# yyssys/MH-SpGEMM

Measured on AMD Instinct MI355X. Metric: GFLOPS (2·flop(A,B)/t) for C=A·A on 16matrix.txt; HBM GB/s vs roofline, higher is better.
Workload: dtype f64; 1 GPU; cant.mtx A*A (synthetic:cant-like), device-resident A -> device-resident sorted C; matrix=cant, rows=62451, nnzA=4325625, nnzC=17508231, parallelism=single GPU

## Files before the change

include/mhspgemm.h:

```cpp
#ifndef MHSPGEMM_H
#define MHSPGEMM_H
#include <stddef.h>
#include <stdint.h>

#ifdef __cplusplus
extern "C" {
#endif

#define MHS_ABI_VERSION 10

typedef enum mhs_status {
    MHS_OK = 0,
    MHS_ERR_HIP = 1,
    MHS_ERR_OOM = 2,
    MHS_ERR_INVALID = 3,
    MHS_ERR_OVERFLOW = 4,
    MHS_ERR_IO = 5
} mhs_status;

typedef struct mhs_csr {
    int32_t M, N, nnz;
    int32_t *ptr;
    int32_t *col;
    double *val;
// ... 4 lines not shown
    double Form_mask_matrix_B;
    double symbolic_binning;
    double Calculate_C_nnz;
    double numeric_binning;
    double Malloc_C_col_val;
    double Numeric;
    double total_ref;
    double total_e2e;
    uint64_t flop;
    int64_t nnzC;
    int32_t sym_bins[16];
    int32_t num_bins[16];
} mhs_timing;

typedef struct mhs_ctx mhs_ctx;

int mhs_ctx_create(mhs_ctx **ctx, int device);
void mhs_ctx_destroy(mhs_ctx *ctx);
const char *mhs_last_error(const mhs_ctx *ctx);
int mhs_ctx_set_stream(mhs_ctx *ctx, void *hip_stream);
int mhs_ctx_trim(mhs_ctx *ctx);

typedef enum mhs_option { MHS_OPT_SYNC = 1, MHS_OPT_NUMERIC_EVENTS = 2, MHS_OPT_MEM_BUDGET = 3,
                           MHS_OPT_TINY_FIRST_ROWS = 4, MHS_OPT_SPECULATE = 5 } mhs_option;
int mhs_ctx_set_option(mhs_ctx *ctx, int option, int value);
long long mhs_ctx_chunked_calls(const mhs_ctx *ctx);
typedef enum mhs_stat { MHS_STAT_CHUNKED = 0, MHS_STAT_SPLIT = 1, MHS_STAT_SYM_FORK = 2, MHS_STAT_NFT = 3,
                        MHS_STAT_NEAR = 4, MHS_STAT_MULTI_STREAM = 5, MHS_STAT_SPEC = 6, MHS_STAT_SPEC_MISS = 7,
                        MHS_STAT_SPEC_SKIPPED = 8 } mhs_stat;
long long mhs_ctx_stat(const mhs_ctx *ctx, int which);
int mhs_ctx_numeric_ms(mhs_ctx *ctx, float *out, int n);

int mhs_probe_conflicts(mhs_ctx *ctx, uint64_t *count);

int mhs_spgemm(mhs_ctx *ctx, const mhs_csr *A, const mhs_csr *B, mhs_csr *C, mhs_timing *t);

typedef struct mhs_values_plan mhs_values_plan;

int mhs_values_plan_create(mhs_ctx *ctx, const mhs_csr *A, const mhs_csr *B, const mhs_csr *C,
                           mhs_values_plan **plan);
int mhs_spgemm_values(mhs_ctx *ctx, mhs_values_plan *plan, const double *Aval, const double *Bval,
                      double *Cval, double *ms);
typedef struct mhs_values_info {
    int32_t rows[8];
    int64_t products, nnzC, plan_bytes;
} mhs_values_info;
int mhs_values_plan_info(const mhs_values_plan *plan, mhs_values_info *info);
// ... 35 lines not shown
```

mh-spgemm_amd/csrc/mhs_api.cpp:

```cpp
#include "mhs_internal.hpp"
#include "mhs_owner.hpp"
#include "../../include/mhspgemm.h"

#include <algorithm>
#include <chrono>
#include <cstdio>
#include <cstdlib>
#include <cstring>
#include <string>
#include <unordered_map>
#include <vector>

using namespace mhs;

struct mhs_ctx {
    int device = 0;
    hipStream_t own_stream = nullptr;
    hipStream_t stream = nullptr;
    std::string err;
    char* ws = nullptr;
    size_t ws_bytes = 0;
    char* gscratch = nullptr;
    size_t gscratch_bytes = 0;
    Stats* h_stats = nullptr;
// ... 28 lines not shown
    std::vector<std::pair<void*, size_t>> pool;
    hipEvent_t stream_ev = nullptr;
    static constexpr int NAUX = 7;
    int num_streams = 4;
    hipStream_t aux[NAUX] = {};
    hipEvent_t fork_ev = nullptr, join_ev[NAUX] = {};
    hipEvent_t split_ev = nullptr;
    struct PlanKey {
        const void* p[6];
        long long M, N, MB, nnzA, nnzB, gen;
        int near, nft, mc_list, pad;
        bool operator==(const PlanKey& o) const { return memcmp(this, &o, sizeof *this) == 0; }
    };
    bool spec = true;
    bool plan_valid = false;
    PlanKey plan_key{};
    Stats plan_h{};
    long long gen = 0;
    int* d_go = nullptr;
    bool spec_fork = false;
    bool spec_fork_rare = true;
    bool fork_common_first = true;
    int spec_nss = mhs_ctx::NAUX + 1;
};

struct mhs_values_plan {
    int device = 0;
    ValPattern pat{};
    long long nnzA = 0, nnzB = 0, nnzC = 0, products = 0;
    char* mem = nullptr;
    size_t mem_bytes = 0;
    int* lists = nullptr;
    int list_off[VAL_NCLASS] = {};
    ValCounts counts{};
    ValPlan plan{};
    hipEvent_t ev[2] = {};
};

namespace {
constexpr int VAL_STATUS_INTS = 8;
}

namespace {

int fail(mhs_ctx* ctx, int code, const std::string& what) {
    if (ctx) ctx->err = what;
// ... 270 lines not shown
    if (rc) return rc;
    memcpy(&h, (const void*)&ctx->pub->stats, sizeof(Stats));
    ctx->stats_zero = true;
    ++ctx->front_passes;
    return MHS_OK;
}

constexpr int NUM_GLOBAL_GRID = 128;
#ifndef MHS_MULTI_FLOP_LOG2
#define MHS_MULTI_FLOP_LOG2 22
#endif

#ifndef MHS_SPLIT_FLOP_LOG2
#define MHS_SPLIT_FLOP_LOG2 24
#endif

int numeric_streams(const mhs_ctx* ctx, const Stats& h) {
    const int nl = numeric_launches(h);
    return (nl >= 3 && h.flop >= (1ull << MHS_MULTI_FLOP_LOG2)) ? std::min(ctx->num_streams, nl) : 1;
}

enum NumPhase { NUM_ALL = 0, NUM_SPEC_A = 1, NUM_SPEC_B = 2 };

NumShape num_shape(const Csr& a, const Csr& b, const Work& w, bool split) {
    return NumShape{a.M, a.nnz, b.nnz, w.bx_on, w.sc_col != nullptr, split, NUM_GLOBAL_GRID};
}

int run_numeric(mhs_ctx* ctx, const Csr& a, const Csr& b, const Work& w, const Stats& h, const mhs_csr& out,
                NumPlan& plan, hipEvent_t ev0 = nullptr, hipEvent_t ev1 = nullptr, int phase = NUM_ALL) {
    hipStream_t s = ctx->stream;
    hipStream_t ss[mhs_ctx::NAUX + 1] = {s};
    int nss = numeric_streams(ctx, h);
    if (w.go) nss = std::min(nss, ctx->spec_nss);
    for (int i = 1; i < nss; ++i) ss[i] = ctx->aux[i - 1];
    const bool first = phase != NUM_SPEC_B, last = phase != NUM_SPEC_A;
    if (phase == NUM_SPEC_B && nss == 1) return MHS_OK;
    if (first && nss > 1 && ev0) MHS_HIP(hipEventRecord(ev0, s));
    if (first && nss > 1) MHS_HIP(hipEventRecord(ctx->fork_ev, s));
    if (first) {
        const bool want_split = nss > 1 && ctx->split && h.flop >= (1ull << MHS_SPLIT_FLOP_LOG2);
        const bool split = want_split && launch_split_bins(w, h, a.M, out.ptr, s, ctx->dense_span_max);
        if (split) MHS_HIP(hipEventRecord(ctx->split_ev, s));
        ctx->stat[MHS_STAT_SPLIT] += split;
        ctx->stat[MHS_STAT_MULTI_STREAM] += nss > 1;
        plan = plan_numeric(h, num_shape(a, b, w, split));
    }
    const NumPointers np{a, b, w, out.ptr, out.col, out.val, ctx->dense_span_max};
    hipError_t fe = hipSuccess;
    bool forked = false;
    int used = 0;
    auto fork = [&]() {
        forked = true;
        for (int i = 1; i < nss && fe == hipSuccess; ++i) fe = hipStreamWaitEvent(ss[i], ctx->fork_ev, 0);
    };
    for (int i = 0; i < plan.n; ++i) {
        const NumLaunch& l = plan.launch[i];
        const int dealt = stream_of(i, nss);
        if (phase == NUM_SPEC_A ? dealt != 0 : phase == NUM_SPEC_B && dealt == 0) continue;
        if (dealt != 0 && !forked) fork();
        const int k = fe == hipSuccess ? dealt : 0;
        used |= 1 << k;
        if (l.after_split && k != 0) (void)hipStreamWaitEvent(ss[k], ctx->split_ev, 0);
        issue_numeric(l, plan.o32, np, ss[k], nss == 1 && i == 0 ? ev0 : nullptr,
                      nss == 1 && i + 1 == plan.n ? ev1 : nullptr);
    }
    if (nss == 1 && plan.n == 0) {
        if (ev0) MHS_HIP(hipEventRecord(ev0, s));
        if (ev1) MHS_HIP(hipEventRecord(ev1, s));
// ... 100 lines not shown
        if (e != hipSuccess) {
            free_cached(ctx);
            (void)hipGetLastError();
            return e == hipErrorOutOfMemory ? fail(ctx, MHS_ERR_OOM, "C itself does not fit the device")
                                            : fail_hip(ctx, e, "allocating C (row-chunked)");
        }
    }
    ctx->c_held = (size_t)(M + 1) * 4 + (size_t)total * 12;
    rc = fit_workspace(Mc1);
    ctx->c_held = 0;
    if (rc) return rc;
    nch = (M + Mc - 1) / Mc;
    long long off = 0;
    int sym[NBINS] = {}, num[NBINS] = {};
    own.queued = true;
    for (int c = 0; c < nch; ++c) {
        const Csr a = view(c);
        const int r0 = c * Mc;
        Work w = make_work(ctx, L, a.M, a.nnz, B->nnz, mc_list);
        rc = front_pass(ctx, a, b, w, out.ptr + r0, c == 0, h);
        if (rc == MHS_OK) rc = ensure_gscratch(ctx, w, h);
        if (rc) return rc;
        if (h.nnzC > 0) {
            const NumPlan p = plan_numeric(h, num_shape(a, b, w, false));
            const NumPointers np{a, b, w, out.ptr + r0, out.col + off, out.val + off, ctx->dense_span_max};
            for (int i = 0; i < p.n; ++i) issue_numeric(p.launch[i], p.o32, np, s, nullptr, nullptr);
        }
        launch_add_offset(out.ptr + r0, a.M + (c == nch - 1 ? 1 : 0), (int)off, s);
        MHS_HIP(hipGetLastError());
        off += h.nnzC;
        for (int i = 1; i < NBINS; ++i) {
            sym[i] += h.sym_count[i];
            num[i] += h.num_count[i];
        }
    }
    MHS_HIP(hipStreamSynchronize(s));
    own.commit(C);
    ++ctx->chunked_calls;
    if (t) {
        mhs_timing tm{};
        tm.total_e2e = tm.total_ref = ms_since(T0);
        tm.flop = flop;
        tm.nnzC = total;
        fill_bins(tm, M, sym, num);
        *t = tm;
    }
    return MHS_OK;
// ... 369 lines not shown
int mhs_ctx_create(mhs_ctx** out, int device) {
    if (!out) return MHS_ERR_INVALID;
    *out = nullptr;
    mhs_ctx* ctx = new mhs_ctx();
    ctx->device = device;
    hipError_t e = hipSetDevice(device);
    if (e == hipSuccess) e = hipStreamCreateWithFlags(&ctx->own_stream, hipStreamNonBlocking);
    if (e == hipSuccess) e = hipHostMalloc((void**)&ctx->h_stats, sizeof(Stats), hipHostMallocDefault);
    if (e == hipSuccess)
        e = hipHostMalloc((void**)&ctx->pub, sizeof(Published), hipHostMallocMapped | hipHostMallocCoherent);
    if (e == hipSuccess) e = hipHostGetDevicePointer((void**)&ctx->d_pub, ctx->pub, 0);
    if (e == hipSuccess) memset(ctx->pub, 0, sizeof(Published));
    for (int i = 0; e == hipSuccess && i < 8; ++i) e = hipEventCreate(&ctx->ev[i]);
    if (e == hipSuccess) e = hipEventCreateWithFlags(&ctx->stream_ev, hipEventDisableTiming);
    if (const char* v = getenv("MHS_NUM_STREAMS")) ctx->num_streams = std::max(1, std::min(atoi(v), mhs_ctx::NAUX + 1));
    if (e == hipSuccess) e = hipEventCreateWithFlags(&ctx->fork_ev, hipEventDisableTiming);
    if (e == hipSuccess) e = hipEventCreateWithFlags(&ctx->split_ev, hipEventDisableTiming);
    for (int i = 0; e == hipSuccess && i + 1 < ctx->num_streams; ++i) {
        e = hipStreamCreateWithFlags(&ctx->aux[i], hipStreamNonBlocking);
        if (e == hipSuccess) e = hipEventCreateWithFlags(&ctx->join_ev[i], hipEventDisableTiming);
    }
    if (e == hipSuccess) e = hipMalloc((void**)&ctx->d_go, 256);
    if (e == hipSuccess) e = init_kernel_attributes();
    if (e != hipSuccess) {
        fprintf(stderr, "mhs_ctx_create: %s\n", hipGetErrorString(e));
        delete ctx;
        return e == hipErrorOutOfMemory ? MHS_ERR_OOM : MHS_ERR_HIP;
    }
    ctx->stream = ctx->own_stream;
    if (const char* e = getenv("MHS_DENSE_SPAN")) ctx->dense_span_max = atoi(e);
    if (getenv("MHS_NO_MCACHE")) ctx->use_mcache = false;
    if (const char* e = getenv("MHS_MC_LIST")) ctx->mc_list = atoi(e) < MC_LIST_MIN ? MC_LIST_MIN : atoi(e);
    if (getenv("MHS_NO_GROUPS")) ctx->groups = false;
    if (getenv("MHS_NO_NEAR")) ctx->near = false;
    if (getenv("MHS_NO_SPLIT")) ctx->split = false;
    if (getenv("MHS_NO_TINY_NUM")) ctx->tiny_num = false;
    if (const char* e = getenv("MHS_NFT_MIN_M")) ctx->nft_min_m = atoll(e);
    if (getenv("MHS_NFT_NO_SLOTS")) ctx->nft_slots = false;
    if (const char* e = getenv("MHS_SYM_FORK")) ctx->sym_fork = atoi(e) != 0;
    if (const char* e = getenv("MHS_SYM_FORK_MIN_M")) ctx->sym_fork_min_m = atoll(e);
    if (const char* e = getenv("MHS_NFT_OTHER_PCT")) ctx->nft_other_pct = atoi(e);
    if (const char* e = getenv("MHS_NFT_AUTO_AVG")) ctx->nft_auto_avg = atoi(e);
    if (const char* e = getenv("MHS_NO_SPEC")) ctx->spec = atoi(e) == 0;
    if (const char* e = getenv("MHS_FORK_ORDER")) ctx->fork_common_first = atoi(e) != 0;
    if (const char* e = getenv("MHS_SPEC_FORK")) {
        ctx->spec_fork = atoi(e) == 1;
        ctx->spec_fork_rare = atoi(e) == 2;
    }
    if (const char* e = getenv("MHS_SPEC_NSS")) ctx->spec_nss = std::max(1, std::min(atoi(e), mhs_ctx::NAUX + 1));
    *out = ctx;
    return MHS_OK;
}

void mhs_ctx_destroy(mhs_ctx* ctx) {
    if (!ctx) return;
    (void)hipSetDevice(ctx->device);
    if (ctx->stream) (void)hipStreamSynchronize(ctx->stream);
    mhs_ctx_trim(ctx);
    if (ctx->stream_ev) (void)hipEventDestroy(ctx->stream_ev);
    if (ctx->fork_ev) (void)hipEventDestroy(ctx->fork_ev);
    if (ctx->split_ev) (void)hipEventDestroy(ctx->split_ev);
    for (int i = 0; i < mhs_ctx::NAUX; ++i) {
        if (ctx->aux[i]) {
            (void)hipStreamSynchronize(ctx->aux[i]);
            (void)hipStreamDestroy(ctx->aux[i]);
        }
        if (ctx->join_ev[i]) (void)hipEventDestroy(ctx->join_ev[i]);
    }
    if (ctx->h_stats) (void)hipHostFree(ctx->h_stats);
    if (ctx->pub) (void)hipHostFree(ctx->pub);
    for (auto& ev : ctx->nev)
// ... 228 lines not shown
    case MHS_OPT_NUMERIC_EVENTS: {
        if (value < 0 || value > 4096) return fail(ctx, MHS_ERR_INVALID, "numeric event ring size out of [0, 4096]");
        MHS_HIP(hipSetDevice(ctx->device));
        MHS_HIP(hipStreamSynchronize(ctx->stream));
        for (auto& ev : ctx->nev) (void)hipEventDestroy(ev);
        ctx->nev.assign(2 * (size_t)value, nullptr);
        for (auto& ev : ctx->nev) MHS_HIP(hipEventCreate(&ev));
        ctx->ncalls = 0;
        return MHS_OK;
    }
    case MHS_OPT_MEM_BUDGET:
        if (value < 0) return fail(ctx, MHS_ERR_INVALID, "memory budget must be >= 0 MiB");
        ctx->mem_budget = (size_t)value << 20;
        ++ctx->gen;
        return MHS_OK;
    case MHS_OPT_SPECULATE:
        ctx->spec = value != 0;
        ctx->plan_valid = false;
        return MHS_OK;
    case MHS_OPT_TINY_FIRST_ROWS:
        ctx->nft_min_m = value;
        ++ctx->gen;
        return MHS_OK;
    default:
        return fail(ctx, MHS_ERR_INVALID, "unknown option");
    }
}

long long mhs_ctx_chunked_calls(const mhs_ctx* ctx) { return ctx ? ctx->chunked_calls : -1; }

long long mhs_ctx_stat(const mhs_ctx* ctx, int which) {
    if (!ctx || which < 0 || which > MHS_STAT_SPEC_SKIPPED) return -1;
    return which == MHS_STAT_CHUNKED ? ctx->chunked_calls : ctx->stat[which];
}

int mhs_ctx_numeric_ms(mhs_ctx* ctx, float* out, int n) {
    if (!ctx || (!out && n > 0)) return -MHS_ERR_INVALID;
    const long long ring = (long long)ctx->nev.size() / 2;
    if (ring == 0) return 0;
    long long have = ctx->ncalls < ring ? ctx->ncalls : ring;
    if (n < have) have = n;
    for (long long i = 0; i < have; ++i) {
        const long long call = ctx->ncalls - have + i;
        const int slot = (int)(call % ring);
        if (hipEventSynchronize(ctx->nev[2 * slot + 1]) != hipSuccess) return -MHS_ERR_HIP;
        float f = 0;
// ... 54 lines not shown
```

mh-spgemm_amd/csrc/mhs_kernels.hip:

```cpp
#include "mhs_internal.hpp"

#include <hip/hip_ext.h>

#include <algorithm>
#include <climits>
#include <cstdlib>
#include <type_traits>

#ifndef MHS_ROW_STAMPS
#define MHS_ROW_STAMPS 0
#endif
constexpr int MHS_RUN_MAX = 3;
constexpr int MHS_RUN_UNROLL = 2;
constexpr int MHS_TILE_UNROLL = 2;
constexpr int MHS_UNROLL = 4;
constexpr int MHS_UNROLL_BLOCK = 8;
constexpr int MHS_NFT_GRID = 4096, MHS_NFT_GRID_BIG = 16384;
constexpr int MHS_TINY_PF = 1;
constexpr int MHS_SYM_WAVE_GRID = 2048;
constexpr int MHS_SYM_WAVE_GRID_BIG = 65536;
constexpr int MHS_VAL_GMIN = 4;
constexpr int MHS_TILE_GMIN = 4;
constexpr int MHS_RUN_GMIN = 8;
constexpr int MHS_MASK_GMAX = 64;
// ... 2785 lines not shown
    const int* rlo;
    const int* rhi;
    const int* ctiles;
    const int* list;
    int count;
    const unsigned char* grp;
    const int* Cptr;
    int* Ccol;
    double* Cval;
    char* gscratch;
    long long gbytes;
    int dense_span_max;
    const unsigned long long* mcache;
    int mc_list, mc_stride;
    int* cursor;
    SpillLists sp;
    int qall;
    const int* ucol;
    const double* uval;
    const int* gna;
    int ubase;
    int wave_bytes;
    const int* go;
};
#define MHS_PLAN_GUARD(args) \
    if ((args).go && *(args).go != 1) return

__device__ __forceinline__ void store_vals(double* __restrict__ dst, const double* src, int n, int rank, int T) {
    for (int r = 2 * rank; r < n; r += 2 * T) {
        if (r + 1 < n) __builtin_nontemporal_store(*(const d2u*)(src + r), (d2u*)(dst + r));
        else st_stream(dst + r, src[r]);
    }
}
__device__ __forceinline__ void store_cols(int* __restrict__ dst, const int* cb, int n, int R, int rank, int T) {
    for (int r = 4 * rank; r < n; r += 4 * T) {
        if (r + 3 < n) {
            const i4a c4 = *(const i4a*)(cb + r);
            for (int g = 0; g < R; ++g) __builtin_nontemporal_store((i4u)c4, (i4u*)(dst + g * n + r));
        } else {
            for (int k = r; k < n; ++k)
                for (int g = 0; g < R; ++g) st_stream(&dst[g * n + k], cb[k]);
        }
    }
}
template <bool DIRECT>
__device__ __forceinline__ void stage_cols(const TileEntry* E, int H, int lo, int* cb, int rank, int T) {
    const int lane = lane_id();
    for (int s0 = rank & ~63; s0 < H; s0 += T) {
        const int s = s0 + lane;
// ... 5 lines not shown
            key = DIRECT ? lo + s : e.key;
            base = e.base;
        }
        const bool big = __popcll(mk) > 8;
        unsigned long long bigs = __ballot(big);
        if (!big) {
            int r = base;
            while (mk) {
                cb[r++] = (key << TILE_SHIFT) + __builtin_ctzll(mk);
                mk &= mk - 1;
            }
        }
        while (bigs) {
            const int src = __builtin_ctzll(bigs);
            bigs &= bigs - 1;
            const uint4 q = *reinterpret_cast<const uint4*>(&E[s0 + src]);
            const unsigned long long m2 = ((unsigned long long)q.y << 32) | q.x;
            const int k2 = DIRECT ? lo + s0 + src : (int)q.w;
            if ((m2 >> lane) & 1ull) cb[(int)q.z + __popcll(m2 & lanemask_lt())] = (k2 << TILE_SHIFT) + lane;
        }
    }
}

template <class Team, bool GLOBALMEM, int MODE, bool GROUPED, bool O32>
__device__ __forceinline__ void num_row_body(const Team& tm, const NumArgs& a, int row, int lo, int span, int t,
                             int c0, int n, int a0, int a1, char* region, int* counter,
                             int4* stage, int R) {
    MHS_BSTAMP0();
    const int H = MODE == NM_HASH ? hash_slots(t) : span;
    const int colbase = lo << TILE_SHIFT;
    TileEntry* E = (TileEntry*)region;
    double* acc = (double*)(region + (long long)H * 16);
    const int nacc = MODE == NM_DENSE ? span * TILE_BITS : n;
    const int tflop = __builtin_amdgcn_readfirstlane(a.rtflop[row]);
    const int stride = GROUPED ? (int)(num_acc_bytes(MODE, span, t, n) / 8) : 0;
    const int nclear = GROUPED ? (R - 1) * stride + nacc : nacc;

    GroupPair gp;
    bool gnear = false;
    int gnw = a1 - a0;
    const int* gcol = a.Acol;
    const double* gval = a.Aval;
    if constexpr (GROUPED) {
        gnear = (__builtin_amdgcn_readfirstlane((int)a.grp[row]) & GRP_NEAR) != 0;
        if (gnear) {
            gnw = __builtin_amdgcn_readfirstlane(a.gna[row]);
            gcol = a.ucol;
            gval = a.uval + 2LL * a0;
        }
        group_pair_a(gp, a0, a0 + gnw, gcol, gval, R, gnw);
    }
    MHS_BSTAMP(0);
    const bool sym_tiny = tiny_class_sym(__builtin_amdgcn_readfirstlane(a.rflop[row]), a1 - a0) >= 0;
    const int lofs = (a.mcache && !sym_tiny && spill_row(span, tflop, t, a.mc_list))
                         ? __builtin_amdgcn_readfirstlane(a.sp.lofs[row])
                         : -1;
    const bool rank_bitmap = MODE == NM_HASH && (Team::size > 64 || t >= 64) &&
                             (long long)((span + 63) >> 6) * 12 + 16 + (long long)t * 4 <=
                                 num_acc_bytes(NM_HASH, span, t, n);
    const bool rank_count = MODE == NM_HASH && !rank_bitmap &&
                            (t <= HASH_CNT_T || (long long)((t + Team::size - 1) / Team::size) * t <= 768);
    bool have_list = false;
    if (MODE != NM_HASH && a.mcache && mcached(span, tflop) && !sym_tiny) {
        for (int s = tm.rank(); s < span; s += Team::size) {
            TileEntry z;
            z.mask = ld_cache(&a.mcache[(size_t)row * a.mc_stride + s]);
            z.base = 0;
            z.key = -1;
            E[s] = z;
        }
        tm.sync();
    } else if (a.mcache && !sym_tiny && (mlisted(span, tflop, t, a.mc_list) || lofs >= 0)) {
        const unsigned long long* slot = lofs >= 0 ? a.sp.mask + lofs : a.mcache + (size_t)row * a.mc_stride;
        const int* skey = lofs >= 0 ? a.sp.key + lofs : reinterpret_cast<const int*>(slot + a.mc_list);
        clear_tiles(tm, E, H);
        if (MODE == NM_HASH && tm.rank() == 0) *counter = 0;
// ... 7 lines not shown
                int sl = hslot(key, H);
                MHS_GUARD_DECL;
                while (atomicCAS(&E[sl].key, -1, key) != -1) {
                    MHS_GUARD(H, 4, key);
                    probe_conflict();
                    sl = hnext(sl, H);
                }
                E[sl].mask = m;
                if (rank_count) reinterpret_cast<int2*>(acc)[r] = make_int2(key, (sl << 8) | __popcll(m));
            }
        }
        have_list = MODE == NM_HASH && rank_count;
        tm.sync();
    } else {
        clear_tiles(tm, E, H);
        if (MODE == NM_HASH && tm.rank() == 0) *counter = 0;
        tm.sync();
        build_tiles(tm, E, MODE != NM_HASH, lo, H, a0, a1, a.Acol, a.bmeta, a.btcol, a.btmask,
                    tflop, stage);
        tm.sync();
    }
    MHS_BSTAMP(1);

    if constexpr (GROUPED) group_pair_meta(gp, a.bmeta);
    if constexpr (MODE != NM_HASH) {
        tm.exclusive_scan(
            span, [&](int i) { return (int)__popcll(E[i].mask); },
            [&](int i, int v) { E[i].base = v; });
    } else if (rank_bitmap) {
        const int nw = (span + 63) >> 6;
        unsigned long long* bm = (unsigned long long*)acc;
        int* wpre = (int*)(bm + nw);
        int* cnt = wpre + ((nw + 3) & ~3);
        for (int i = tm.rank(); i < nw; i += Team::size) bm[i] = 0ull;
        tm.sync();
        for (int s = tm.rank(); s < H; s += Team::size) {
            const int key = E[s].key;
            if (key != -1) atomicOr(&bm[(key - lo) >> 6], 1ull << ((key - lo) & 63));
        }
        tm.sync();
        tm.exclusive_scan(
            nw, [&](int i) { return (int)__popcll(bm[i]); }, [&](int i, int v) { wpre[i] = v; });
        tm.sync();
        auto rank_of = [&](int key) {
            const int d = key - lo;
            return wpre[d >> 6] + (int)__popcll(bm[d >> 6] & ((1ull << (d & 63)) - 1));
// ... 42 lines not shown
        }
    } else {
        unsigned long long* S = (unsigned long long*)acc;
        const int P = next_pow2(t);
        for (int s = tm.rank(); s < H; s += Team::size) {
            const int key = E[s].key;
            if (key != -1) {
                const int idx = atomicAdd(counter, 1);
                S[idx] = ((unsigned long long)(unsigned)key << 32) | (unsigned)s;
            }
        }
        for (int i = t + tm.rank(); i < P; i += Team::size) S[i] = ~0ull;
        tm.sync();
        team_bitonic(tm, S, P);
        tm.exclusive_scan(
            t, [&](int e) { return (int)__popcll(E[(int)(unsigned)S[e]].mask); },
            [&](int e, int v) { E[(int)(unsigned)S[e]].base = v; });
    }
    tm.sync();
    MHS_BSTAMP(2);
    for (int r = tm.rank(); r < nclear; r += Team::size) acc[r] = 0.0;
    tm.sync();
    MHS_BSTAMP(3);

    {
        const Accum<GLOBALMEM, MODE, O32> f{E, acc, lo, H, colbase, a.Bcol, a.Bval, a.ubase};
        if constexpr (GROUPED) {
            const int nAr = a1 - a0;
            const int avg = nAr > 0 ? (__builtin_amdgcn_readfirstlane(a.rflop[row]) + nAr - 1) / nAr : 1;
            for_products_group(gp, a0, a0 + gnw, gcol, gval, a.bmeta, avg, f, R, gnw, stride);
        } else {
            walk_products(tm, a0, a1, a.Acol, a.Aval, a.bmeta, false, a.rflop[row], f, stage);
        }
    }
    tm.sync();
    MHS_BSTAMP(4);

    if constexpr (MODE == NM_DENSE) {
        const int lane = lane_id();
        const int nw = Team::size / 64, wv = tm.rank() >> 6;
        for (int s = wv; s < span; s += nw) {
            const TileEntry e = E[s];
            if ((e.mask >> lane) & 1ull) {
                const int pos = c0 + e.base + __popcll(e.mask & lanemask_lt());
                for (int g = 0; g < (GROUPED ? R : 1); ++g) {
                    st_part(&a.Ccol[pos + g * n], colbase + (s << TILE_SHIFT) + lane);
                    st_part(&a.Cval[pos + g * n], acc[g * stride + (s << TILE_SHIFT) + lane]);
                }
            }
        }
    } else {
        for (int g = 0; g < (GROUPED ? R : 1); ++g)
// ... 172 lines not shown
                  RankAccum<false, O32>{bm, wpre, msk, kb, acc, lo, a.Bcol, a.Bval}, stage);
    tm.sync();
    MHS_STAMP(4);
    store_vals(a.Cval + c0, acc, n, tm.rank(), T);
    tm.sync();
    int* cb = (int*)acc;
    for (int r = tm.rank(); r < t; r += T) {
        unsigned long long m = msk[r];
        const int2 e = kb[r];
        int b = e.y;
        while (m) {
            cb[b++] = (e.x << TILE_SHIFT) + __builtin_ctzll(m);
            m &= m - 1;
        }
    }
    tm.sync();
    store_cols(a.Ccol + c0, cb, n, 1, tm.rank(), T);
    tm.sync();
    MHS_STAMP(5);
}

enum NumModes : int { MODES_ALL = 0, MODES_NOHASH = 1, MODES_HASH = 2 };

struct NumRow {
    int row, lo, hi, t, c0, n, a0, a1;
};
template <class Team, bool GLOBALMEM, bool GROUPED = false, int MODES = MODES_ALL, bool O32 = false>
__device__ __forceinline__ void num_row_s(const Team& tm, const NumArgs& a, const NumRow& r, char* region,
                                          int* counter, int4* stage, int R = 1);
template <class Team, bool GLOBALMEM, bool GROUPED = false, int MODES = MODES_ALL, bool O32 = false>
__device__ __forceinline__ void num_row(const Team& tm, const NumArgs& a, int row, char* region, int* counter,
                        int4* stage, int R = 1) {
    NumRow r;
    r.row = row;
    r.lo = __builtin_amdgcn_readfirstlane(a.rlo[row]);
    r.hi = __builtin_amdgcn_readfirstlane(a.rhi[row]);
    r.t = __builtin_amdgcn_readfirstlane(a.ctiles[row]);
    r.c0 = __builtin_amdgcn_readfirstlane(a.Cptr[row]);
    r.n = __builtin_amdgcn_readfirstlane(a.Cptr[row + 1]) - r.c0;
    r.a0 = __builtin_amdgcn_readfirstlane(a.Aptr[row]);
    r.a1 = __builtin_amdgcn_readfirstlane(a.Aptr[row + 1]);
    num_row_s<Team, GLOBALMEM, GROUPED, MODES, O32>(tm, a, r, region, counter, stage, R);
}
template <class Team, bool GLOBALMEM, bool GROUPED, int MODES, bool O32>
__device__ __forceinline__ void num_row_s(const Team& tm, const NumArgs& a, const NumRow& r, char* region,
                                          int* counter, int4* stage, int R) {
    const int row = r.row, lo = r.lo, hi = r.hi, t = r.t, c0 = r.c0, n = r.n, a0 = r.a0, a1 = r.a1;
    const int span = hi - lo + 1;
    const int mode = num_mode(span, t, n, a.dense_span_max);
    if constexpr (MODES == MODES_HASH) {
        num_row_body<Team, GLOBALMEM, NM_HASH, GROUPED, O32>(tm, a, row, lo, span, t, c0, n, a0, a1, region, counter, stage, R);
        return;
    }
    if (mode == NM_DENSE)
        num_row_body<Team, GLOBALMEM, NM_DENSE, GROUPED, O32>(tm, a, row, lo, span, t, c0, n, a0, a1, region, counter, stage, R);
    else if (MODES == MODES_NOHASH || mode == NM_DIRECT)
        num_row_body<Team, GLOBALMEM, NM_DIRECT, GROUPED, O32>(tm, a, row, lo, span, t, c0, n, a0, a1, region, counter, stage, R);
    else
        num_row_body<Team, GLOBALMEM, NM_HASH, GROUPED, O32>(tm, a, row, lo, span, t, c0, n, a0, a1, region, counter, stage, R);
}


template <int BYTES, bool GROUPED, bool HASH, bool O32>
__device__ __forceinline__ void num_wave_rows(const NumArgs& a, int bid = -1, int nb = -1) {
    extern __shared__ __attribute__((aligned(16))) char smem[];
    if (bid < 0) {
        bid = (int)blockIdx.x;
        nb = (int)gridDim.x;
    }
    const int w = threadIdx.x >> 6;
    char* reg = smem + w * (GROUPED && a.wave_bytes > 0 ? a.wave_bytes : BYTES);
    WaveTeam tm;
    auto one = [&](int li) {
        const int row = __builtin_amdgcn_readfirstlane(a.list[li]);
        MHS_FLIGHT_ROW(row, li);
        if constexpr (GROUPED)
            num_row<WaveTeam, false, true, MODES_ALL, O32>(tm, a, row, reg + WAVE_HDR, (int*)reg, nullptr,
                                                         __builtin_amdgcn_readfirstlane((int)a.grp[row]) & GRP_RMASK);
        else
            num_row<WaveTeam, false, false, HASH ? MODES_HASH : MODES_NOHASH, O32>(tm, a, row, reg + WAVE_HDR,
                                                                             (int*)reg, nullptr);
    };
    constexpr bool guided = BYTES == NUM_W16_BYTES && HASH;
    if (guided && a.qall) {
        WaveQueue q(a.cursor, a.count, 1);
        for (int li; q.next(li);) one(li);
    } else if (guided && (gridDim.x & 7) == 0) {
        const int g = (int)(blockIdx.x & 7);
        const int begin = (int)((long long)a.count * g / 8), end = (int)((long long)a.count * (g + 1) / 8);
        const int split = begin + (int)((long long)(end - begin) * MHS_GUIDED_STATIC / 8);
        const int stride = (int)(gridDim.x >> 3) * WPB;
        for (int li = begin + (int)(blockIdx.x >> 3) * WPB + w; li < split; li += stride) one(li);
        int* cur = a.cursor + g * CURSOR_STRIDE;
        for (;;) {
            int t = 0;
            if (lane_id() == 0) t = atomicAdd(cur, 1);
            const int li = split + __builtin_amdgcn_readfirstlane(t);
            MHS_FLIGHT_TAKE(li);
            if (li >= end) break;
            one(li);
        }
    } else {
        for (RowWalk rw(a.count, WPB, w, bid, nb); rw.first < rw.end; rw.first += rw.stride) one(rw.first);
    }
// ... 743 lines not shown
    a.rhi = w.rhi;
    a.ctiles = w.ctiles;
    a.Cptr = p.Cptr;
    a.Ccol = p.Ccol;
    a.Cval = p.Cval;
    a.gscratch = (char*)w.gscratch;
    a.grp = w.grp;
    a.sp = w.spill;
    a.ucol = w.ucol;
    a.uval = w.uval;
    a.gna = w.gna;
    a.go = w.go;
    if (w.bx_on) {
        a.ubase = p.B.nnz;
        a.Bcol = w.bx_col;
        a.Bval = w.bx_val;
    }
    a.list = l.list_bin == LIST_SPLIT ? w.split_list + l.list_off : w.bin_list + (long long)(l.list_bin - 1) * p.A.M;
    a.count = l.count;
    a.cursor = w.cursors + l.slot * 8 * CURSOR_STRIDE;
    a.gbytes = l.gbytes;
    a.qall = l.qall;
    a.wave_bytes = l.wave_bytes;
    return a;
}

TinyArgs tiny_args(const NumPointers& p, const NumLaunch& l) {
    TinyArgs t{};
    t.M = p.A.M;
    t.Aptr = p.A.ptr;
    t.Acol = p.A.col;
    t.Aval = p.A.val;
    t.bmeta = p.w.bmeta;
    t.Bcol = p.B.col;
    t.Bval = p.B.val;
    t.Cptr = p.Cptr;
    t.Ccol = p.Ccol;
    t.Cval = p.Cval;
    t.rlo = p.w.rlo;
    t.go = p.w.go;
    if (l.list_bin == LIST_CLASSES) {
        t.list = p.w.bin_list;
    } else {
        t.count = l.count;
        t.bin = l.list_bin;
        t.list = p.w.bin_list + (long long)(l.list_bin - 1) * p.A.M;
// ... 72 lines not shown
```

mh-spgemm_amd/csrc/mhs_numplan.hpp:

```cpp
#pragma once
#include "mhs_shape.hpp"

namespace mhs {

constexpr int MHS_NUM_WS_GRID = 4096;
constexpr int MHS_TINY64_GRID = 4096;
constexpr int MHS_NUM_W16H_GRID = 2048;
constexpr int MHS_COPY_CAP_BIG = 65536;
constexpr int MHS_NFT_BIG_M = 1 << 22;
constexpr int MHS_NUM_WSH_BIG = (1 << 21);
constexpr int MHS_NUM_WSH_BIG_GRID = 65536;
constexpr int MHS_NUM_WSX_GRID = 16384;
constexpr int MHS_DYN16_MAX = 32768;

inline int round8(long long x, int cap) {
    long long g = x < cap ? x : cap;
    if (g < 8) g = 8;
    return (int)((g + 7) / 8 * 8);
}
inline int block_lds(int need, int budget, int T) {
    if (need <= 0) return budget;
    const int b = (block_hdr(T) + need + 2047) & ~2047;
    return b < budget ? b : budget;
}
// ... 24 lines not shown
};

struct TinyFused {
    int nclass;
    int c[4];
    int count[4];
    int blk0[5];
};

enum : int { LIST_SPLIT = 0, LIST_CLASSES = -1 };
struct NumLaunch {
    int kernel;
    int variant;
    int grid, block, lds;
    int list_bin;
    int list_off;
    int count, slot;
    int wave_bytes;
    int gbytes;
    int qall;
    int hash_blocks;
    int after_split;
    TinyFused fused;
};

constexpr int NUM_PLAN_MAX = 16;
struct NumPlan {
    int n;
    int o32;
    NumLaunch launch[NUM_PLAN_MAX];
};

struct NumShape {
    int M, nnzA, nnzB;
    int bx_on;
    int slot_rows;
    int split;
    int global_grid;
};

inline NumPlan plan_numeric(const Stats& h, const NumShape& sh) {
    NumPlan p{};
    p.o32 = (long long)sh.nnzB + (sh.bx_on ? 3LL * sh.nnzA : 0) < (1LL << 29);
    auto add = [&](int kernel, int bin, int count, long long blocks, int cap, int threads, int lds) -> NumLaunch& {
        NumLaunch& l = p.launch[p.n < NUM_PLAN_MAX ? p.n++ : NUM_PLAN_MAX - 1];
        l = NumLaunch{};
        l.kernel = kernel;
        l.grid = round8(blocks, cap);
        l.block = threads;
        l.lds = lds;
        l.list_bin = bin;
        l.count = count;
        l.slot = bin > 0 ? bin : 0;
        return l;
    };
    auto wave_bin = [&](int kernel, int bin, int cap, int wave_bytes) -> NumLaunch& {
        const int count = h.num_count[bin];
        return add(kernel, bin, count, (count + WPB - 1) / WPB, cap, 256, WPB * wave_bytes);
    };
    auto fused = [&](bool ranges, int lanes(int)) {
        TinyFused f{};
// ... 73 lines not shown
        const int count = h.num_count[NUM_TINY + c];
        if (count <= 0) continue;
        const int per = 256 / tiny_w(c);
        add(NK_TINY64, NUM_TINY + c, count, (count + per - 1) / per, MHS_TINY64_GRID, 256, 256 * tiny_k(c) * 8).variant = c;
    }
    static_assert(tiny_w(3) <= 32 && tiny_k(0) <= TINY_FUSED_KMAX && tiny_k(1) <= TINY_FUSED_KMAX &&
                      tiny_k(2) <= TINY_FUSED_KMAX && tiny_k(3) <= TINY_FUSED_KMAX && tiny_w(4) == 64,
                  "classes 0..3 fuse (W <= 32, K <= TINY_FUSED_KMAX)");
    if (!sh.slot_rows) {
        const TinyFused f = fused(true, [](int c) { return tiny_w(c); });
        if (f.nclass > 0) {
            int rows = 0;
            for (int k = 0; k < f.nclass; ++k) rows += f.count[k];
            const int blocks = f.blk0[f.nclass];
            add(NK_TINY_SMALL, LIST_CLASSES, rows, blocks, blocks, 256, 256 * TINY_FUSED_KMAX * 8).fused = f;
        }
    }
    if (h.num_count[NUM_W16G] > 0) {
        const int wb = wave_region(h.num_wave_need[1], NUM_W16_BYTES);
        wave_bin(NK_GROUP16, NUM_W16G, 2048, wb).wave_bytes = wb;
    }
    if (h.num_count[NUM_WSG] > 0) {
        const int wb = wave_region(h.num_wave_need[0], NUM_WSG_BYTES);
        wave_bin(NK_GROUP, NUM_WSG, MHS_NUM_WS_GRID, wb).wave_bytes = wb;
    }
    if (h.num_count[NUM_WS] > 0) wave_bin(NK_DIRECT, NUM_WS, MHS_NUM_WSX_GRID, NUM_WS_BYTES);
    return p;
}

inline int numeric_launches(const Stats& h) {
    int n = 0, small = 0;
    for (int b = 1; b < NUM_NB; ++b) {
        if (h.num_count[b] <= 0) continue;
        if (b >= NUM_TINY && b < NUM_TINY + 4) small = 1;
        else ++n;
    }
    return n + small + block_split_on(h, 0) + block_split_on(h, 1);
}

inline int stream_of(int i, int n) { return n > 1 ? i % n : 0; }

}
```

mh-spgemm_amd/mhspgemm/_lib.py:

```python
from __future__ import annotations

import ctypes
import os
import re
from pathlib import Path

HERE = Path(__file__).resolve().parent
LIB_PATH = Path(os.environ["MHS_LIB"]) if os.environ.get("MHS_LIB") else HERE / "libmhspgemm.so"
HEADER = HERE.parent.parent / "include" / "mhspgemm.h"

MHS_OK = 0
MHS_ERR_HIP = 1
MHS_ERR_OOM = 2
MHS_ERR_INVALID = 3
MHS_ERR_OVERFLOW = 4
MHS_ERR_IO = 5

MHS_OPT_SYNC = 1
MHS_OPT_NUMERIC_EVENTS = 2
MHS_OPT_MEM_BUDGET = 3
MHS_OPT_TINY_FIRST_ROWS = 4
MHS_OPT_SPECULATE = 5

STATUS_NAMES = {0: "MHS_OK", 1: "MHS_ERR_HIP", 2: "MHS_ERR_OOM", 3: "MHS_ERR_INVALID",
                4: "MHS_ERR_OVERFLOW", 5: "MHS_ERR_IO"}


class mhs_csr(ctypes.Structure):
    _fields_ = [("M", ctypes.c_int32), ("N", ctypes.c_int32), ("nnz", ctypes.c_int32),
                ("ptr", ctypes.c_void_p), ("col", ctypes.c_void_p), ("val", ctypes.c_void_p)]


class mhs_timing(ctypes.Structure):
    _fields_ = [("mem_alloc", ctypes.c_double), ("Form_mask_matrix_B", ctypes.c_double),
                ("symbolic_binning", ctypes.c_double), ("Calculate_C_nnz", ctypes.c_double),
                ("numeric_binning", ctypes.c_double), ("Malloc_C_col_val", ctypes.c_double),
                ("Numeric", ctypes.c_double), ("total_ref", ctypes.c_double),
                ("total_e2e", ctypes.c_double), ("flop", ctypes.c_uint64), ("nnzC", ctypes.c_int64),
                ("sym_bins", ctypes.c_int32 * 16), ("num_bins", ctypes.c_int32 * 16)]


class mhs_host_csr(ctypes.Structure):
    _fields_ = [("M", ctypes.c_int32), ("N", ctypes.c_int32), ("nnz", ctypes.c_int32),
                ("ptr", ctypes.c_void_p), ("col", ctypes.c_void_p), ("val", ctypes.c_void_p),
                ("is_symmetric", ctypes.c_int32)]
# ... 121 lines not shown
```

Baseline: 2580 GFLOPS.

## Add XCD-grouped persistent walk with row-metadata prefetch for grouped numeric kernel

The grouped wave-numeric kernel now runs as a persistent, XCD-aware walk. Each of eight groups takes a contiguous slice of the row list, processes most rows statically, and hands the tail out through per-group atomic cursors. The grid is capped at the estimated number of resident blocks, based on CU count and LDS use. The next row's list entry and scalar metadata are prefetched across lanes and read back with readlane while the current row is processed. The aim is to cut launch and tail imbalance and hide per-row metadata load latency, at the cost of extra atomics, added register pressure, and reliance on an assumption about how blocks map to XCDs.

```diff
diff --git a/include/mhspgemm.h b/include/mhspgemm.h
--- a/include/mhspgemm.h
+++ b/include/mhspgemm.h
@@ -50,7 +50,7 @@
 int mhs_ctx_trim(mhs_ctx *ctx);
 
 typedef enum mhs_option { MHS_OPT_SYNC = 1, MHS_OPT_NUMERIC_EVENTS = 2, MHS_OPT_MEM_BUDGET = 3,
-                           MHS_OPT_TINY_FIRST_ROWS = 4, MHS_OPT_SPECULATE = 5 } mhs_option;
+                           MHS_OPT_TINY_FIRST_ROWS = 4, MHS_OPT_SPECULATE = 5, MHS_OPT_GROUP_GRID = 6 } mhs_option;
 int mhs_ctx_set_option(mhs_ctx *ctx, int option, int value);
 long long mhs_ctx_chunked_calls(const mhs_ctx *ctx);
 typedef enum mhs_stat { MHS_STAT_CHUNKED = 0, MHS_STAT_SPLIT = 1, MHS_STAT_SYM_FORK = 2, MHS_STAT_NFT = 3,
diff --git a/mh-spgemm_amd/csrc/mhs_api.cpp b/mh-spgemm_amd/csrc/mhs_api.cpp
--- a/mh-spgemm_amd/csrc/mhs_api.cpp
+++ b/mh-spgemm_amd/csrc/mhs_api.cpp
@@ -74,6 +74,8 @@
     bool spec_fork_rare = true;
     bool fork_common_first = true;
     int spec_nss = mhs_ctx::NAUX + 1;
+    int cus = 0;
+    int group_cap = 0;
 };
 
 struct mhs_values_plan {
@@ -390,8 +392,8 @@
 
 enum NumPhase { NUM_ALL = 0, NUM_SPEC_A = 1, NUM_SPEC_B = 2 };
 
-NumShape num_shape(const Csr& a, const Csr& b, const Work& w, bool split) {
-    return NumShape{a.M, a.nnz, b.nnz, w.bx_on, w.sc_col != nullptr, split, NUM_GLOBAL_GRID};
+NumShape num_shape(const mhs_ctx* ctx, const Csr& a, const Csr& b, const Work& w, bool split) {
+    return NumShape{a.M, a.nnz, b.nnz, w.bx_on, w.sc_col != nullptr, split, NUM_GLOBAL_GRID, ctx->cus, ctx->group_cap};
 }
 
 int run_numeric(mhs_ctx* ctx, const Csr& a, const Csr& b, const Work& w, const Stats& h, const mhs_csr& out,
@@ -411,7 +413,7 @@
         if (split) MHS_HIP(hipEventRecord(ctx->split_ev, s));
         ctx->stat[MHS_STAT_SPLIT] += split;
         ctx->stat[MHS_STAT_MULTI_STREAM] += nss > 1;
-        plan = plan_numeric(h, num_shape(a, b, w, split));
+        plan = plan_numeric(h, num_shape(ctx, a, b, w, split));
     }
     const NumPointers np{a, b, w, out.ptr, out.col, out.val, ctx->dense_span_max};
     hipError_t fe = hipSuccess;
@@ -558,7 +560,7 @@
         if (rc == MHS_OK) rc = ensure_gscratch(ctx, w, h);
         if (rc) return rc;
         if (h.nnzC > 0) {
-            const NumPlan p = plan_numeric(h, num_shape(a, b, w, false));
+            const NumPlan p = plan_numeric(h, num_shape(ctx, a, b, w, false));
             const NumPointers np{a, b, w, out.ptr + r0, out.col + off, out.val + off, ctx->dense_span_max};
             for (int i = 0; i < p.n; ++i) issue_numeric(p.launch[i], p.o32, np, s, nullptr, nullptr);
         }
@@ -974,6 +976,7 @@
     }
     if (e == hipSuccess) e = hipMalloc((void**)&ctx->d_go, 256);
     if (e == hipSuccess) e = init_kernel_attributes();
+    if (e == hipSuccess) e = hipDeviceGetAttribute(&ctx->cus, hipDeviceAttributeMultiprocessorCount, device);
     if (e != hipSuccess) {
         fprintf(stderr, "mhs_ctx_create: %s\n", hipGetErrorString(e));
         delete ctx;
@@ -999,6 +1002,9 @@
         ctx->spec_fork = atoi(e) == 1;
         ctx->spec_fork_rare = atoi(e) == 2;
     }
+    if (const char* e = getenv("MHS_GROUP_WALK"))
+        if (atoi(e) == 0) ctx->cus = 0;
+    if (const char* e = getenv("MHS_GROUP_GRID")) ctx->group_cap = std::max(0, atoi(e));
     if (const char* e = getenv("MHS_SPEC_NSS")) ctx->spec_nss = std::max(1, std::min(atoi(e), mhs_ctx::NAUX + 1));
     *out = ctx;
     return MHS_OK;
@@ -1273,6 +1279,11 @@
         ctx->nft_min_m = value;
         ++ctx->gen;
         return MHS_OK;
+    case MHS_OPT_GROUP_GRID:
+        if (value < 0) return fail(ctx, MHS_ERR_INVALID, "grouped grid cap must be >= 0 blocks");
+        ctx->group_cap = value;
+        ++ctx->gen;
+        return MHS_OK;
     default:
         return fail(ctx, MHS_ERR_INVALID, "unknown option");
     }
diff --git a/mh-spgemm_amd/csrc/mhs_groupwalk.hpp b/mh-spgemm_amd/csrc/mhs_groupwalk.hpp
--- /dev/null
+++ b/mh-spgemm_amd/csrc/mhs_groupwalk.hpp
@@ -0,0 +1,44 @@
+#pragma once
+#include "mhs_shape.hpp"
+
+namespace mhs {
+
+constexpr int GROUP_NONE = -1;
+constexpr int GROUP_XCDS = 8;
+#ifndef MHS_GROUP_DYN_ROUNDS
+#define MHS_GROUP_DYN_ROUNDS 1
+#endif
+constexpr int GROUP_DYN_ROUNDS = MHS_GROUP_DYN_ROUNDS;
+
+__host__ __device__ inline int group_begin(int count, int g) { return (int)((long long)count * g / GROUP_XCDS); }
+
+struct GroupWalk {
+    int begin, split, end;
+    int waves;
+};
+__host__ __device__ inline GroupWalk group_walk(int count, int g, int blocks) {
+    GroupWalk w;
+    w.begin = group_begin(count, g);
+    w.end = group_begin(count, g + 1);
+    w.waves = blocks / GROUP_XCDS * WPB;
+    const int rounds = w.waves > 0 ? (w.end - w.begin) / w.waves : 0;
+    w.split = w.begin + (rounds > GROUP_DYN_ROUNDS ? rounds - GROUP_DYN_ROUNDS : 0) * w.waves;
+    return w;
+}
+__host__ __device__ inline int group_static_first(const GroupWalk& w, int j) {
+    return w.begin + j < w.split ? w.begin + j : GROUP_NONE;
+}
+__host__ __device__ inline int group_static_next(const GroupWalk& w, int li) {
+    return li + w.waves < w.split ? li + w.waves : GROUP_NONE;
+}
+__host__ __device__ inline int group_take(const GroupWalk& w, int ticket) {
+    return (unsigned)ticket < (unsigned)(w.end - w.split) ? w.split + ticket : GROUP_NONE;
+}
+
+__host__ __device__ inline int group_resident_blocks(int cus, int wave_bytes) {
+    const int by_lds = wave_bytes > 0 ? LDS_MAX_C / (WPB * wave_bytes) : 4;
+    const int per_cu = by_lds < 4 ? (by_lds < 1 ? 1 : by_lds) : 4;
+    return cus * per_cu;
+}
+
+}
diff --git a/mh-spgemm_amd/csrc/mhs_kernels.hip b/mh-spgemm_amd/csrc/mhs_kernels.hip
--- a/mh-spgemm_amd/csrc/mhs_kernels.hip
+++ b/mh-spgemm_amd/csrc/mhs_kernels.hip
@@ -2831,9 +2831,84 @@
     int ubase;
     int wave_bytes;
     const int* go;
+    int cursor_walk;
 };
 #define MHS_PLAN_GUARD(args) \
     if ((args).go && *(args).go != 1) return
+
+struct NumRow {
+    int row, lo, hi, t, c0, n, a0, a1;
+};
+struct NoNext {
+    static constexpr bool kOn = false;
+    int tflop, rflop, grp, gna;
+    __device__ __forceinline__ void take() {}
+    __device__ __forceinline__ void head() {}
+    __device__ __forceinline__ void scalars() {}
+};
+struct GroupNext {
+    enum : int { K_LO, K_HI, K_T, K_C0, K_C1, K_A0, K_A1, K_TFLOP, K_RFLOP, K_GNA, K_GRP, K_ROW };
+    static constexpr bool kOn = true;
+    const NumArgs& a;
+    int* cur;
+    GroupWalk gw;
+    int li;
+    bool dyn;
+    int v;
+    NumRow r;
+    int tflop, rflop, grp, gna;
+    __device__ __forceinline__ bool static_left() const { return !dyn && group_static_next(gw, li) != GROUP_NONE; }
+    __device__ __forceinline__ void take() {
+        if (cur && !static_left()) {
+            v = 0;
+            if (lane_id() == 0) v = atomicAdd(cur, 1);
+        }
+    }
+    __device__ __forceinline__ void head() {
+        int nli = GROUP_NONE;
+        if (static_left()) {
+            nli = group_static_next(gw, li);
+        } else if (cur) {
+            dyn = true;
+            nli = group_take(gw, __builtin_amdgcn_readfirstlane(v));
+            MHS_FLIGHT_TAKE(nli);
+        }
+        li = nli;
+        v = -1;
+        if (nli != GROUP_NONE) {
+            int z;
+            asm volatile("v_mov_b32 %0, 0" : "=v"(z));
+            v = a.list[nli + z];
+        }
+    }
+    __device__ __forceinline__ void scalars() {
+        const int row = __builtin_amdgcn_readfirstlane(v);
+        if (row < 0) return;
+        const int k = lane_id();
+        const int* p = k == K_LO ? a.rlo : k == K_HI ? a.rhi : k == K_T ? a.ctiles : k <= K_C1 ? a.Cptr
+                     : k <= K_A1 ? a.Aptr : k == K_TFLOP ? a.rtflop : k == K_RFLOP ? a.rflop : a.gna;
+        int x = row;
+        if (k < K_GNA || (k == K_GNA && a.gna)) x = p[row + (k == K_C1 || k == K_A1)];
+        if (k == K_GRP) x = a.grp[row];
+        v = x;
+    }
+    __device__ __forceinline__ bool advance() {
+        r.row = __builtin_amdgcn_readlane(v, K_ROW);
+        if (r.row < 0) return false;
+        r.lo = __builtin_amdgcn_readlane(v, K_LO);
+        r.hi = __builtin_amdgcn_readlane(v, K_HI);
+        r.t = __builtin_amdgcn_readlane(v, K_T);
+        r.c0 = __builtin_amdgcn_readlane(v, K_C0);
+        r.n = __builtin_amdgcn_readlane(v, K_C1) - r.c0;
+        r.a0 = __builtin_amdgcn_readlane(v, K_A0);
+        r.a1 = __builtin_amdgcn_readlane(v, K_A1);
+        tflop = __builtin_amdgcn_readlane(v, K_TFLOP);
+        rflop = __builtin_amdgcn_readlane(v, K_RFLOP);
+        gna = __builtin_amdgcn_readlane(v, K_GNA);
+        grp = __builtin_amdgcn_readlane(v, K_GRP);
+        return true;
+    }
+};
 
 __device__ __forceinline__ void store_vals(double* __restrict__ dst, const double* src, int n, int rank, int T) {
     for (int r = 2 * rank; r < n; r += 2 * T) {
@@ -2885,17 +2960,18 @@
     }
 }
 
-template <class Team, bool GLOBALMEM, int MODE, bool GROUPED, bool O32>
+template <class Team, bool GLOBALMEM, int MODE, bool GROUPED, bool O32, class NX = NoNext>
 __device__ __forceinline__ void num_row_body(const Team& tm, const NumArgs& a, int row, int lo, int span, int t,
                              int c0, int n, int a0, int a1, char* region, int* counter,
-                             int4* stage, int R) {
+                             int4* stage, int R, NX* nx = nullptr) {
     MHS_BSTAMP0();
     const int H = MODE == NM_HASH ? hash_slots(t) : span;
     const int colbase = lo << TILE_SHIFT;
     TileEntry* E = (TileEntry*)region;
     double* acc = (double*)(region + (long long)H * 16);
     const int nacc = MODE == NM_DENSE ? span * TILE_BITS : n;
-    const int tflop = __builtin_amdgcn_readfirstlane(a.rtflop[row]);
+    const int tflop = NX::kOn ? nx->tflop : __builtin_amdgcn_readfirstlane(a.rtflop[row]);
+    auto rflop = [&]() { return NX::kOn ? nx->rflop : __builtin_amdgcn_readfirstlane(a.rflop[row]); };
     const int stride = GROUPED ? (int)(num_acc_bytes(MODE, span, t, n) / 8) : 0;
     const int nclear = GROUPED ? (R - 1) * stride + nacc : nacc;
 
@@ -2905,16 +2981,17 @@
     const int* gcol = a.Acol;
     const double* gval = a.Aval;
     if constexpr (GROUPED) {
-        gnear = (__builtin_amdgcn_readfirstlane((int)a.grp[row]) & GRP_NEAR) != 0;
+        gnear = ((NX::kOn ? nx->grp : __builtin_amdgcn_readfirstlane((int)a.grp[row])) & GRP_NEAR) != 0;
         if (gnear) {
-            gnw = __builtin_amdgcn_readfirstlane(a.gna[row]);
+            gnw = NX::kOn ? nx->gna : __builtin_amdgcn_readfirstlane(a.gna[row]);
             gcol = a.ucol;
             gval = a.uval + 2LL * a0;
         }
         group_pair_a(gp, a0, a0 + gnw, gcol, gval, R, gnw);
     }
+    if constexpr (NX::kOn) nx->take();
     MHS_BSTAMP(0);
-    const bool sym_tiny = tiny_class_sym(__builtin_amdgcn_readfirstlane(a.rflop[row]), a1 - a0) >= 0;
+    const bool sym_tiny = tiny_class_sym(rflop(), a1 - a0) >= 0;
     const int lofs = (a.mcache && !sym_tiny && spill_row(span, tflop, t, a.mc_list))
                          ? __builtin_amdgcn_readfirstlane(a.sp.lofs[row])
                          : -1;
@@ -2968,6 +3045,7 @@
     }
     MHS_BSTAMP(1);
 
+    if constexpr (NX::kOn) nx->head();
     if constexpr (GROUPED) group_pair_meta(gp, a.bmeta);
     if constexpr (MODE != NM_HASH) {
         tm.exclusive_scan(
@@ -3056,12 +3134,13 @@
     for (int r = tm.rank(); r < nclear; r += Team::size) acc[r] = 0.0;
     tm.sync();
     MHS_BSTAMP(3);
+    if constexpr (NX::kOn) nx->scalars();
 
     {
         const Accum<GLOBALMEM, MODE, O32> f{E, acc, lo, H, colbase, a.Bcol, a.Bval, a.ubase};
         if constexpr (GROUPED) {
             const int nAr = a1 - a0;
-            const int avg = nAr > 0 ? (__builtin_amdgcn_readfirstlane(a.rflop[row]) + nAr - 1) / nAr : 1;
+            const int avg = nAr > 0 ? (rflop() + nAr - 1) / nAr : 1;
             for_products_group(gp, a0, a0 + gnw, gcol, gval, a.bmeta, avg, f, R, gnw, stride);
         } else {
             walk_products(tm, a0, a1, a.Acol, a.Aval, a.bmeta, false, a.rflop[row], f, stage);
@@ -3280,12 +3359,9 @@
 
 enum NumModes : int { MODES_ALL = 0, MODES_NOHASH = 1, MODES_HASH = 2 };
 
-struct NumRow {
-    int row, lo, hi, t, c0, n, a0, a1;
-};
-template <class Team, bool GLOBALMEM, bool GROUPED = false, int MODES = MODES_ALL, bool O32 = false>
+template <class Team, bool GLOBALMEM, bool GROUPED = false, int MODES = MODES_ALL, bool O32 = false, class NX = NoNext>
 __device__ __forceinline__ void num_row_s(const Team& tm, const NumArgs& a, const NumRow& r, char* region,
-                                          int* counter, int4* stage, int R = 1);
+                                          int* counter, int4* stage, int R = 1, NX* nx = nullptr);
 template <class Team, bool GLOBALMEM, bool GROUPED = false, int MODES = MODES_ALL, bool O32 = false>
 __device__ __forceinline__ void num_row(const Team& tm, const NumArgs& a, int row, char* region, int* counter,
                         int4* stage, int R = 1) {
@@ -3300,22 +3376,22 @@
     r.a1 = __builtin_amdgcn_readfirstlane(a.Aptr[row + 1]);
     num_row_s<Team, GLOBALMEM, GROUPED, MODES, O32>(tm, a, r, region, counter, stage, R);
 }
-template <class Team, bool GLOBALMEM, bool GROUPED, int MODES, bool O32>
+template <class Team, bool GLOBALMEM, bool GROUPED, int MODES, bool O32, class NX>
 __device__ __forceinline__ void num_row_s(const Team& tm, const NumArgs& a, const NumRow& r, char* region,
-                                          int* counter, int4* stage, int R) {
+                                          int* counter, int4* stage, int R, NX* nx) {
     const int row = r.row, lo = r.lo, hi = r.hi, t = r.t, c0 = r.c0, n = r.n, a0 = r.a0, a1 = r.a1;
     const int span = hi - lo + 1;
     const int mode = num_mode(span, t, n, a.dense_span_max);
     if constexpr (MODES == MODES_HASH) {
-        num_row_body<Team, GLOBALMEM, NM_HASH, GROUPED, O32>(tm, a, row, lo, span, t, c0, n, a0, a1, region, counter, stage, R);
+        num_row_body<Team, GLOBALMEM, NM_HASH, GROUPED, O32>(tm, a, row, lo, span, t, c0, n, a0, a1, region, counter, stage, R, nx);
         return;
     }
     if (mode == NM_DENSE)
-        num_row_body<Team, GLOBALMEM, NM_DENSE, GROUPED, O32>(tm, a, row, lo, span, t, c0, n, a0, a1, region, counter, stage, R);
+        num_row_body<Team, GLOBALMEM, NM_DENSE, GROUPED, O32>(tm, a, row, lo, span, t, c0, n, a0, a1, region, counter, stage, R, nx);
     else if (MODES == MODES_NOHASH || mode == NM_DIRECT)
-        num_row_body<Team, GLOBALMEM, NM_DIRECT, GROUPED, O32>(tm, a, row, lo, span, t, c0, n, a0, a1, region, counter, stage, R);
+        num_row_body<Team, GLOBALMEM, NM_DIRECT, GROUPED, O32>(tm, a, row, lo, span, t, c0, n, a0, a1, region, counter, stage, R, nx);
     else
-        num_row_body<Team, GLOBALMEM, NM_HASH, GROUPED, O32>(tm, a, row, lo, span, t, c0, n, a0, a1, region, counter, stage, R);
+        num_row_body<Team, GLOBALMEM, NM_HASH, GROUPED, O32>(tm, a, row, lo, span, t, c0, n, a0, a1, region, counter, stage, R, nx);
 }
 
 
@@ -3329,15 +3405,42 @@
     const int w = threadIdx.x >> 6;
     char* reg = smem + w * (GROUPED && a.wave_bytes > 0 ? a.wave_bytes : BYTES);
     WaveTeam tm;
+    if constexpr (GROUPED) {
+        GroupNext nx{a};
+        nx.dyn = false;
+        if (a.cursor_walk && (nb & 7) == 0) {
+            const int g = bid & 7;
+            nx.gw = group_walk(a.count, g, nb);
+            nx.cur = a.cursor + g * CURSOR_STRIDE;
+            nx.li = nx.gw.begin + (bid >> 3) * WPB + w - nx.gw.waves;
+        } else {
+            nx.cur = nullptr;
+            if ((nb & 7) == 0) {
+                const int g = bid & 7;
+                nx.gw.waves = (nb >> 3) * WPB;
+                nx.gw.split = nx.gw.end = group_begin(a.count, g + 1);
+                nx.li = group_begin(a.count, g) + (bid >> 3) * WPB + w - nx.gw.waves;
+            } else {
+                nx.gw.waves = nb * WPB;
+                nx.gw.split = nx.gw.end = a.count;
+                nx.li = bid * WPB + w - nx.gw.waves;
+            }
+        }
+        nx.take();
+        nx.head();
+        nx.scalars();
+        while (nx.advance()) {
+            MHS_FLIGHT_ROW(nx.r.row, nx.li);
+            num_row_s<WaveTeam, false, true, MODES_ALL, O32>(tm, a, nx.r, reg + WAVE_HDR, (int*)reg, nullptr,
+                                                           nx.grp & GRP_RMASK, &nx);
+        }
+        return;
+    }
     auto one = [&](int li) {
         const int row = __builtin_amdgcn_readfirstlane(a.list[li]);
         MHS_FLIGHT_ROW(row, li);
-        if constexpr (GROUPED)
-            num_row<WaveTeam, false, true, MODES_ALL, O32>(tm, a, row, reg + WAVE_HDR, (int*)reg, nullptr,
-                                                         __builtin_amdgcn_readfirstlane((int)a.grp[row]) & GRP_RMASK);
-        else
-            num_row<WaveTeam, false, false, HASH ? MODES_HASH : MODES_NOHASH, O32>(tm, a, row, reg + WAVE_HDR,
-                                                                             (int*)reg, nullptr);
+        num_row<WaveTeam, false, false, HASH ? MODES_HASH : MODES_NOHASH, O32>(tm, a, row, reg + WAVE_HDR, (int*)reg,
+                                                                         nullptr);
     };
     constexpr bool guided = BYTES == NUM_W16_BYTES && HASH;
     if (guided && a.qall) {
@@ -4127,6 +4230,7 @@
     a.gbytes = l.gbytes;
     a.qall = l.qall;
     a.wave_bytes = l.wave_bytes;
+    a.cursor_walk = l.cursor_walk;
     return a;
 }
 
diff --git a/mh-spgemm_amd/csrc/mhs_numplan.hpp b/mh-spgemm_amd/csrc/mhs_numplan.hpp
--- a/mh-spgemm_amd/csrc/mhs_numplan.hpp
+++ b/mh-spgemm_amd/csrc/mhs_numplan.hpp
@@ -1,4 +1,5 @@
 #pragma once
+#include "mhs_groupwalk.hpp"
 #include "mhs_shape.hpp"
 
 namespace mhs {
@@ -70,6 +71,7 @@
     int hash_blocks;
     int after_split;
     TinyFused fused;
+    int cursor_walk;
 };
 
 constexpr int NUM_PLAN_MAX = 16;
@@ -85,6 +87,8 @@
     int slot_rows;
     int split;
     int global_grid;
+    int cus = 0;
+    int group_cap = 0;
 };
 
 inline NumPlan plan_numeric(const Stats& h, const NumShape& sh) {
@@ -204,7 +208,14 @@
     }
     if (h.num_count[NUM_WSG] > 0) {
         const int wb = wave_region(h.num_wave_need[0], NUM_WSG_BYTES);
-        wave_bin(NK_GROUP, NUM_WSG, MHS_NUM_WS_GRID, wb).wave_bytes = wb;
+        NumLaunch& l = wave_bin(NK_GROUP, NUM_WSG, MHS_NUM_WS_GRID, wb);
+        l.wave_bytes = wb;
+        const int resident = sh.group_cap > 0 ? sh.group_cap : sh.cus > 0 ? group_resident_blocks(sh.cus, wb) : 0;
+        const int blocks = (l.count + WPB - 1) / WPB;
+        if (resident > 0 && (blocks > resident || sh.group_cap > 0)) {
+            l.grid = round8(blocks, resident < MHS_NUM_WS_GRID ? resident : MHS_NUM_WS_GRID);
+            l.cursor_walk = 1;
+        }
     }
     if (h.num_count[NUM_WS] > 0) wave_bin(NK_DIRECT, NUM_WS, MHS_NUM_WSX_GRID, NUM_WS_BYTES);
     return p;
diff --git a/mh-spgemm_amd/mhspgemm/_lib.py b/mh-spgemm_amd/mhspgemm/_lib.py
--- a/mh-spgemm_amd/mhspgemm/_lib.py
+++ b/mh-spgemm_amd/mhspgemm/_lib.py
@@ -21,6 +21,7 @@
 MHS_OPT_MEM_BUDGET = 3
 MHS_OPT_TINY_FIRST_ROWS = 4
 MHS_OPT_SPECULATE = 5
+MHS_OPT_GROUP_GRID = 6
 
 STATUS_NAMES = {0: "MHS_OK", 1: "MHS_ERR_HIP", 2: "MHS_ERR_OOM", 3: "MHS_ERR_INVALID",
                 4: "MHS_ERR_OVERFLOW", 5: "MHS_ERR_IO"}
```

Result: faster. 2608 GFLOPS, median of 6 (+1.1%).
